# qiaobeibei/PPO-RL-Satellite

Hardware: NVIDIA B200
Metric: rk4_env_steps_per_sec (higher is better)
Workload: dtype f64

## Files before the change

### ppo-rl-satellite_b200/csrc/env_step.cu

```cuda
#include "sat_math.cuh"
#include "../../include/satb200.h"
#include <cmath>

namespace {

using namespace sat;

constexpr int kBlock = 128;
constexpr int kEnvsPerBlock = kBlock / 2;
constexpr int kFrontBlock = 64;
#ifndef SAT_FINISH_MINB
#define SAT_FINISH_MINB 7
#endif
constexpr int kFinishMinBlocks = SAT_FINISH_MINB;
constexpr int kObs = 18;
constexpr int kStatDims = 19;
constexpr int kWsHeader = 256;

SAT_DEV double shfl1(double v) { return __shfl_xor_sync(0xffffffffu, v, 1); }
SAT_DEV int shfl1(int v) { return __shfl_xor_sync(0xffffffffu, v, 1); }

SAT_DEV double clip16(double a) { return a < -1.6 ? -1.6 : (a > 1.6 ? 1.6 : a); }

__host__ __device__ inline int64_t ws_disprev_offset() { return kWsHeader; }
__host__ __device__ inline int64_t ws_partials_offset(int64_t n) { return kWsHeader + ((n * 8 + 255) / 256) * 256; }

struct Lane {
    double r[3], v[3];
    double a[3];
    double fuel_own;
    double dis_prev;
};

template <typename ActT>
SAT_DEV void load_and_gate(const SatEnvState& st, const SatEnvParams& p, const ActT* __restrict__ pa,
                           const ActT* __restrict__ ea, int64_t e, int craft, Lane& L, bool do_impulse,
                           const ActT* raw = nullptr ) {
// ... 40 lines not shown
#pragma unroll
    for (int k = 0; k < 3; ++k) { L.r[k] = y6[k]; L.v[k] = y6[3 + k]; }
}

SAT_DEV void propagate_rk4(const SatEnvParams& p, Lane& L) {
    double X[3], V[3];
#pragma unroll
    for (int k = 0; k < 3; ++k) { X[k] = p.r_cw[k] + L.r[k]; V[k] = p.v_cw[k] + L.v[k]; }
    const Rk4Consts c = make_rk4_consts(p.h, p.mu, p.re, p.j2);
    if (p.j2 != 0.0) {
#pragma unroll 1
        for (int s = 0; s < p.substeps; ++s) rk4_step<true>(X, V, c);
    } else {
#pragma unroll 1
        for (int s = 0; s < p.substeps; ++s) rk4_step<false>(X, V, c);
    }
#pragma unroll
    for (int k = 0; k < 3; ++k) { L.r[k] = X[k] - p.r_cw[k]; L.v[k] = V[k] - p.v_cw[k]; }
}

template <typename ActT, bool OBS>
__global__ void __launch_bounds__(kFrontBlock, 14)
env_front_rk4_kernel(const SatEnvState st, const ActT* __restrict__ pa, const ActT* __restrict__ ea,
                     double* __restrict__ dis_prev_out, float* __restrict__ obs_early,
                     float* __restrict__ pa_copy, float* __restrict__ ea_copy, const __grid_constant__ SatEnvParams p) {
    const int64_t tid = (int64_t)blockIdx.x * kFrontBlock + threadIdx.x;
    const int64_t env_raw = tid >> 1;
    const int craft = (int)(tid & 1);
    const bool valid = env_raw < st.n;
    const int64_t e = valid ? env_raw : st.n - 1;
    Lane L;
    if (OBS) {
        ActT raw[3];
        const ActT* act = craft ? ea : pa;
#pragma unroll
        for (int k = 0; k < 3; ++k) raw[k] = act[e * 3 + k];
        if (valid) {
            float* dc = craft ? ea_copy : pa_copy;
#pragma unroll
            for (int k = 0; k < 3; ++k) dc[e * 3 + k] = (float)raw[k];
        }
        load_and_gate(st, p, pa, ea, e, craft, L, true, raw);
    } else {
        load_and_gate(st, p, pa, ea, e, craft, L, true);
    }
    propagate_rk4(p, L);
    if (valid) {
        const int64_t ld = st.ld;
        const int base = craft * 6;
#pragma unroll
        for (int k = 0; k < 3; ++k) { st.state[(base + k) * ld + e] = L.r[k]; st.state[(base + 3 + k) * ld + e] = L.v[k]; }
        st.state[(SAT_COL_FUEL_C + craft) * ld + e] = L.fuel_own;
        if (craft == 0) dis_prev_out[e] = L.dis_prev;
    }
    if (OBS) {
        double P[3], Pv[3], E[3], Ev[3], d[3];
#pragma unroll
        for (int k = 0; k < 3; ++k) {
            const double o_r = shfl1(L.r[k]), o_v = shfl1(L.v[k]);
            P[k] = craft == 0 ? L.r[k] : o_r;  Pv[k] = craft == 0 ? L.v[k] : o_v;
            E[k] = craft == 0 ? o_r : L.r[k];  Ev[k] = craft == 0 ? o_v : L.v[k];
            d[k] = __dsub_rn(P[k], E[k]);
        }
        const double dis = norm3(d);
        const int count_new = st.istate[SAT_ICOL_COUNT * st.ld + e] + 1;
        const bool done = (dis <= p.d_capture) || (count_new >= p.max_episode_steps);
        if (done && p.auto_reset) {
#pragma unroll
            for (int k = 0; k < 3; ++k) { P[k] = p.reset_p[k]; E[k] = p.reset_e[k]; Pv[k] = 0.0; Ev[k] = 0.0; }
        }
        if (valid) {
            float* o = obs_early + e * kObs + craft * 9;
            if (craft == 0) {
#pragma unroll
                for (int k = 0; k < 3; ++k) { o[k] = (float)__dsub_rn(P[k], E[k]); o[3 + k] = (float)__dsub_rn(Pv[k], Ev[k]); o[6 + k] = (float)P[k]; }
            } else {
#pragma unroll
// ... 42 lines not shown
#endif
template <bool EXACT = true>
SAT_DEV void queue_run(SolveQueue& q) {
    const int total = q.count;
    int task = -1;
    Hybrd1<PFaiT<EXACT>> hs;
    if ((threadIdx.x >> 5) < SAT_SOLVE_WARPS)
    for (;;) {
        if (task < 0) {
            const int t = atomicAdd(&q.next, 1);
            if (t < total) {
                task = t;
                PFaiT<EXACT> f; f.A = q.A[t]; f.sth = q.sth[t]; f.dvm = q.dvm[t];
                hs.init_warm(f, dz_guess(q.guess[t]), q.trig[q.guess[t]]);
            } else task = total;
        }
        const bool active = task < total;
        if (!__any_sync(0xffffffffu, active)) break;
        if (active && hs.step()) { q.alpha[task] = hs.x; task = -1; }
    }
    __syncthreads();
}

template <bool FUSED, typename ActT, int MINB, bool EXACT>
__global__ void __launch_bounds__(kBlock, MINB)
env_step_kernel(const SatEnvState st, const ActT* __restrict__ pa, const ActT* __restrict__ ea,
                const int32_t* __restrict__ count_override, float* __restrict__ obs_f32,
                double* __restrict__ obs_f64, double* __restrict__ term_obs_f64,
                double* __restrict__ reward_out, uint8_t* __restrict__ done_out,
                const double* __restrict__ dis_prev_in, double* __restrict__ partials,
                unsigned int* __restrict__ ticket, const __grid_constant__ SatEnvParams p) {
    union SharedBlock { SolveQueue queue; double tile_term[kEnvsPerBlock][kObs]; __device__ SharedBlock() {} };
    __shared__ SharedBlock shm;
    __shared__ double tile[kEnvsPerBlock][kStatDims];
    SolveQueue& queue = shm.queue;
    double (&tile_term)[kEnvsPerBlock][kObs] = shm.tile_term;
    queue_init<EXACT>(queue);

    const int64_t tid = (int64_t)blockIdx.x * kBlock + threadIdx.x;
    const int64_t env_raw = tid >> 1;
    const int craft = (int)(tid & 1);
    const bool valid = env_raw < st.n;
    const int64_t e = valid ? env_raw : st.n - 1;
    const int64_t ld = st.ld;
    double* __restrict__ S = st.state;
    int32_t* __restrict__ I = st.istate;
    if (ticket && blockIdx.x == 0 && threadIdx.x == 0) *ticket = 0u;

    Lane L;
    load_and_gate(st, p, pa, ea, e, craft, L, FUSED);
    if (FUSED) propagate_cw(p, L);
    else L.dis_prev = dis_prev_in[e];
    const int dz_stale = I[SAT_ICOL_DZ * ld + e];
    const int count = I[SAT_ICOL_COUNT * ld + e];
    int err = I[SAT_ICOL_ERR * ld + e];
    const double ret = S[SAT_COL_RET * ld + e];

    double P[3], Pv[3], E[3], Ev[3], d[3];
#pragma unroll
    for (int k = 0; k < 3; ++k) {
        const double o_r = shfl1(L.r[k]), o_v = shfl1(L.v[k]);
        P[k] = craft == 0 ? L.r[k] : o_r;  Pv[k] = craft == 0 ? L.v[k] : o_v;
        E[k] = craft == 0 ? o_r : L.r[k];  Ev[k] = craft == 0 ? o_v : L.v[k];
        d[k] = __dsub_rn(P[k], E[k]);
    }
    const double dis = norm3(d);
    const int count_new = count_override ? count_override[e] : count + 1;
    const bool captured = dis <= p.d_capture;
    const bool timeout = count_new >= p.max_episode_steps;
    const bool done = captured || timeout;
    const double fuel_oth = shfl1(L.fuel_own);
    const double fuel_c = craft == 0 ? L.fuel_own : fuel_oth;
    double pa_gated[3];
#pragma unroll
    for (int k = 0; k < 3; ++k) { const double o = shfl1(L.a[k]); pa_gated[k] = craft == 0 ? L.a[k] : o; }

    const int le = threadIdx.x >> 1;
    const bool reset_now = done && p.auto_reset;
    const int64_t env0 = (int64_t)blockIdx.x * kEnvsPerBlock;
    const int64_t rem = st.n - env0;
    const int rows = (int)(rem < kEnvsPerBlock ? rem : kEnvsPerBlock);
    {
        double Po[3], Pvo[3], Eo[3], Evo[3];
#pragma unroll
        for (int k = 0; k < 3; ++k) {
            Po[k] = reset_now ? p.reset_p[k] : P[k];  Pvo[k] = reset_now ? 0.0 : Pv[k];
            Eo[k] = reset_now ? p.reset_e[k] : E[k];  Evo[k] = reset_now ? 0.0 : Ev[k];
        }
        if (craft == 0) {
#pragma unroll
            for (int k = 0; k < 3; ++k) { tile[le][k] = __dsub_rn(Po[k], Eo[k]); tile[le][3 + k] = __dsub_rn(Pvo[k], Evo[k]); tile[le][6 + k] = Po[k]; }
        } else {
#pragma unroll
            for (int k = 0; k < 3; ++k) { tile[le][9 + k] = Pvo[k]; tile[le][12 + k] = Eo[k]; tile[le][15 + k] = Evo[k]; }
        }
        __syncthreads();
        const int total = rows * kObs;
        for (int idx = threadIdx.x; idx < total; idx += kBlock) {
            const int row = idx / kObs, col = idx - row * kObs;
            const double val = tile[row][col];
            if (obs_f32) obs_f32[env0 * kObs + idx] = (float)val;
            if (obs_f64) obs_f64[env0 * kObs + idx] = val;
        }
    }

    const bool need_dz = !done && !p.skip_danger_zone && p.flag != 2;
    DzNode nd;
    {
        double Ri[3], Vi[3];
#pragma unroll
        for (int k = 0; k < 3; ++k) { Ri[k] = __dadd_rn(p.r_cw[k], L.r[k]); Vi[k] = __dadd_rn(p.v_cw[k], L.v[k]); }
        dz_prepare<EXACT>(craft, need_dz, Ri, Vi, fuel_c, p.u_grav, nd);
    }
    int slot0, slot1;
    double alpha0, alpha1;
    queue_push(queue, nd, slot0, slot1, alpha0, alpha1);
    queue_run<EXACT>(queue);
    if (slot0 >= 0) alpha0 = queue.alpha[slot0];
    if (slot1 >= 0) alpha1 = queue.alpha[slot1];
    __syncthreads();
    const int dz_eval = dz_finalize<EXACT>(need_dz, nd, alpha0, alpha1, nullptr);
    int dz_new = dz_stale;
    if (need_dz) {
        if (dz_eval >= 0) dz_new = dz_eval;
        else { dz_new = 0; err = 1; }
    }

    double reward = 0.0, cos_a = 0.0, cos_b = 0.0;
    if (p.flag == 2) reward = 0.0;
    else if (captured) reward = (p.flag == 0) ? 100.0 : -150.0;
    else if (timeout) reward = (p.flag == 0) ? 0.0 : 100.0;
    else {
        const bool pv4_on = pa_gated[0] != 0.0 && pa_gated[1] != 0.0 && pa_gated[2] != 0.0;
        double u1[3], w1[3], u2[3], w2[3];
#pragma unroll
        for (int k = 0; k < 3; ++k) {
            u1[k] = craft == 0 ? P[k] : d[k];   w1[k] = craft == 0 ? E[k] : Pv[k];
            u2[k] = craft == 0 ? Pv[k] : d[k];  w2[k] = craft == 0 ? Ev[k] : (pv4_on ? pa_gated[k] : Pv[k]);
        }
        const double ca = cosine3(u1, w1);
        double cb = cosine3(u2, w2);
        if (craft == 1) cb = pv4_on ? -cb : 0.0;
        cos_a = ca; cos_b = cb;
    }
    const double oth_a = shfl1(cos_a), oth_b = shfl1(cos_b);
    if (!captured && !timeout && p.flag != 2) {
        const double pv1 = craft == 0 ? cos_a : oth_a, pv2 = craft == 0 ? cos_b : oth_b;
        const double pv3 = craft == 0 ? oth_a : cos_a, pv4 = craft == 0 ? oth_b : cos_b;
        const double ra = (dis < L.dis_prev) ? 1.0 : -1.0;
        const double rb = (p.d_capture <= dis && dis <= 4.0 * p.d_capture) ? -1.0 : -2.0;
        const double rc = (dz_new == 0) ? -1.0 : dz_new * 0.5;
        double rr = __dadd_rn(__dadd_rn(ra, rb), rc);
        rr = __dadd_rn(rr, pv1);
        rr = __dadd_rn(rr, __dmul_rn(0.6, pv2));
        rr = __dadd_rn(rr, __dmul_rn(0.2, pv3));
        rr = __dadd_rn(rr, __dmul_rn(2.0, pv4));
        reward = (p.flag == 0) ? rr : -rr;
    }
    const double ret_new = __dadd_rn(__dmul_rn(p.gamma, ret), reward);

    if (term_obs_f64) {
        if (craft == 0) {
#pragma unroll
            for (int k = 0; k < 3; ++k) { tile_term[le][k] = d[k]; tile_term[le][3 + k] = __dsub_rn(Pv[k], Ev[k]); tile_term[le][6 + k] = P[k]; }
        } else {
#pragma unroll
            for (int k = 0; k < 3; ++k) { tile_term[le][9 + k] = Pv[k]; tile_term[le][12 + k] = E[k]; tile_term[le][15 + k] = Ev[k]; }
        }
    }

    int int_state_new = 0, count_store = count_new;
    if (reset_now) {
#pragma unroll
        for (int k = 0; k < 3; ++k) {
            P[k] = p.reset_p[k]; E[k] = p.reset_e[k]; Pv[k] = 0.0; Ev[k] = 0.0;
            L.r[k] = craft == 0 ? P[k] : E[k]; L.v[k] = 0.0;
        }
        int_state_new = 1; count_store = 0;
    }

    if (valid) {
        const int base = craft * 6;
        if (FUSED || reset_now) {
#pragma unroll
            for (int k = 0; k < 3; ++k) { S[(base + k) * ld + e] = L.r[k]; S[(base + 3 + k) * ld + e] = L.v[k]; }
        }
        if (FUSED) S[(SAT_COL_FUEL_C + craft) * ld + e] = L.fuel_own;
        if (craft == 0) {
            S[SAT_COL_DIS * ld + e] = dis;
            S[SAT_COL_RET * ld + e] = done ? 0.0 : ret_new;
            I[SAT_ICOL_DZ * ld + e] = dz_new;
            I[SAT_ICOL_COUNT * ld + e] = count_store;
            reward_out[e] = reward;
            done_out[e] = done ? 1 : 0;
        } else {
            I[SAT_ICOL_INTSTATE * ld + e] = int_state_new;
            I[SAT_ICOL_ERR * ld + e] = err;
        }
    }

    if (craft == 0) tile[le][18] = ret_new;
    __syncthreads();
    if (term_obs_f64) {
        const int total = rows * kObs;
        for (int idx = threadIdx.x; idx < total; idx += kBlock) {
            const int row = idx / kObs, col = idx - row * kObs;
            term_obs_f64[env0 * kObs + idx] = tile_term[row][col];
        }
    }
    if (partials && threadIdx.x < kStatDims) {
        const int dim = threadIdx.x;
        double sum = 0.0;
        for (int row = 0; row < rows; ++row) sum += tile[row][dim];
        const double mean = sum / rows;
        double m2 = 0.0;
        for (int row = 0; row < rows; ++row) { double t = tile[row][dim] - mean; m2 += t * t; }
        partials[((int64_t)blockIdx.x * kStatDims + dim) * 2 + 0] = mean;
        partials[((int64_t)blockIdx.x * kStatDims + dim) * 2 + 1] = m2;
    }
}

__global__ void __launch_bounds__(kBlock)
danger_zone_kernel(const double* __restrict__ rv, const double* __restrict__ dv, int64_t n, double u_grav,
                   int32_t* __restrict__ count_out, double* __restrict__ debug_out) {
    __shared__ SolveQueue queue;
    queue_init(queue);
    const int64_t tid = (int64_t)blockIdx.x * kBlock + threadIdx.x;
    const int64_t env_raw = tid >> 1;
    const int craft = (int)(tid & 1);
    const bool valid = env_raw < n;
    const int64_t e = valid ? env_raw : n - 1;
    double Ri[3], Vi[3];
#pragma unroll
    for (int k = 0; k < 3; ++k) { Ri[k] = rv[e * 12 + craft * 6 + k]; Vi[k] = rv[e * 12 + craft * 6 + 3 + k]; }
    DzNode nd;
    dz_prepare(craft, true, Ri, Vi, dv[e], u_grav, nd);
    int slot0, slot1;
    double alpha0, alpha1;
    queue_push(queue, nd, slot0, slot1, alpha0, alpha1);
    queue_run(queue);
    if (slot0 >= 0) alpha0 = queue.alpha[slot0];
    if (slot1 >= 0) alpha1 = queue.alpha[slot1];
    DzDebug dbg = {0, 0, 0, 0, 0, 0, 0, 0};
    const int dz = dz_finalize(true, nd, alpha0, alpha1, debug_out ? &dbg : nullptr);
// ... 181 lines not shown
        double P[3], Pv[3], E[3], Ev[3], o[kObs];
#pragma unroll
        for (int k = 0; k < 3; ++k) {
            P[k] = st.state[(SAT_COL_P + k) * ld + e]; Pv[k] = st.state[(SAT_COL_PV + k) * ld + e];
            E[k] = st.state[(SAT_COL_E + k) * ld + e]; Ev[k] = st.state[(SAT_COL_EV + k) * ld + e];
        }
#pragma unroll
        for (int k = 0; k < 3; ++k) {
            o[k] = __dsub_rn(P[k], E[k]); o[3 + k] = __dsub_rn(Pv[k], Ev[k]);
            o[6 + k] = P[k]; o[9 + k] = Pv[k]; o[12 + k] = E[k]; o[15 + k] = Ev[k];
        }
#pragma unroll
        for (int j = 0; j < kObs; ++j) {
            double v = o[j];
            if (obs_stats) v = (v - obs_stats[1 + j]) / (obs_stats[1 + 2 * kObs + j] + 1e-8);
            tile[threadIdx.x * kObs + j] = (float)v;
        }
    }
    __syncthreads();
    const int64_t rem = st.n - e0;
    const int total = (int)(rem < kObsNormEnvs ? rem : kObsNormEnvs) * kObs;
    for (int idx = threadIdx.x; idx < total; idx += kObsNormEnvs) obs_f32[e0 * kObs + idx] = tile[idx];
}

constexpr int kNormRows = 128;

__global__ void __launch_bounds__(kNormRows)
norm_partial_kernel(const double* __restrict__ x, int64_t n, int dim, double* __restrict__ partials,
                    unsigned int* __restrict__ ticket) {
    __shared__ double tile[kNormRows * 32];
    if (blockIdx.x == 0 && threadIdx.x == 0) *ticket = 0u;
    const int64_t row0 = (int64_t)blockIdx.x * kNormRows;
    const int64_t rem = n - row0;
    const int rows = (int)(rem < kNormRows ? rem : kNormRows);
    const int total = rows * dim;
    for (int idx = threadIdx.x; idx < total; idx += kNormRows) tile[idx] = x[row0 * dim + idx];
    __syncthreads();
    if (threadIdx.x < dim) {
        const int d = threadIdx.x;
        double sum = 0.0;
        for (int r = 0; r < rows; ++r) sum += tile[r * dim + d];
        const double mean = sum / rows;
        double m2 = 0.0;
        for (int r = 0; r < rows; ++r) { double t = tile[r * dim + d] - mean; m2 += t * t; }
        partials[((int64_t)blockIdx.x * dim + d) * 2 + 0] = mean;
        partials[((int64_t)blockIdx.x * dim + d) * 2 + 1] = m2;
    }
}
// ... 7 lines not shown
    const double y = (x[idx] - mean) / (sd + 1e-8);
    if (out64) out64[idx] = y;
    if (out32) out32[idx] = (float)y;
}

int check_state(const SatEnvState* st) {
    if (!st || !st->state || !st->istate) return SAT_ERR_NULL;
    if (st->n <= 0 || st->ld < st->n || (st->ld & 1)) return SAT_ERR_SIZE;
    if (((uintptr_t)st->state & 15) || ((uintptr_t)st->istate & 15)) return SAT_ERR_SIZE;
    return SAT_OK;
}

inline int launch_status() {
    cudaError_t e = cudaGetLastError();
    return e == cudaSuccess ? SAT_OK : (int)e;
}

}

extern "C" {

int64_t sat_workspace_bytes(int64_t n) {
    if (n <= 0) return kWsHeader;
    int64_t nb_env = (n + kEnvsPerBlock - 1) / kEnvsPerBlock;
    int64_t nb_norm = (n + kNormRows - 1) / kNormRows;
    int64_t a = nb_env * kStatDims * 2 * (int64_t)sizeof(double);
    int64_t b = nb_norm * 32 * 2 * (int64_t)sizeof(double);
    return ws_partials_offset(n) + (a > b ? a : b);
}

void sat_env_default_params(SatEnvParams* p) {
    if (!p) return;
    SatEnvParams q = {};
    q.mode = SAT_MODE_CW; q.flag = 0; q.max_episode_steps = 1000; q.auto_reset = 1;
    q.action_dtype = SAT_ACT_F32; q.substeps = 100; q.skip_danger_zone = 0;
    q.d_capture = 100000.0; q.d_range = 100000.0;
    q.gamma = 0.99;
    q.h = 1.0; q.mu = 3.986e14; q.re = 6378137.0; q.j2 = 0.00108263;
    q.r_cw[0] = 27098000.0; q.r_cw[1] = 32306000.0; q.r_cw[2] = 0.0;
    q.v_cw[0] = -2350.0; q.v_cw[1] = 1970.0; q.v_cw[2] = 0.0;
    q.u_grav = 3.986e14;
    q.reset_p[0] = 200000.0; q.reset_e[0] = 18000.0;
    *p = q;
}

int sat_env_init(const SatEnvState* st, double fuel_c, double fuel_t, const SatEnvParams* p, void* stream) {
    int rc = check_state(st);
    if (rc) return rc;
    if (!p) return SAT_ERR_NULL;
    const int threads = 256;
    const unsigned blocks = (unsigned)((st->n + threads - 1) / threads);
// ... 14 lines not shown
int sat_env_observe_norm(const SatEnvState* st, const double* obs_stats, float* obs_f32, void* stream) {
    int rc = check_state(st);
    if (rc) return rc;
    if (!obs_f32) return SAT_ERR_NULL;
    const unsigned blocks = (unsigned)((st->n + kObsNormEnvs - 1) / kObsNormEnvs);
    env_observe_norm_kernel<<<blocks, kObsNormEnvs, 0, (cudaStream_t)stream>>>(*st, obs_stats, obs_f32);
    return launch_status();
}

int sat_env_observe(const SatEnvState* st, float* obs_f32, double* obs_f64, void* stream) {
    int rc = check_state(st);
    if (rc) return rc;
    if (!obs_f32 && !obs_f64) return SAT_ERR_NULL;
    const int threads = 256;
    const int64_t total = st->n * kObs;
    const unsigned blocks = (unsigned)((total + threads - 1) / threads);
    env_observe_kernel<<<blocks, threads, 0, (cudaStream_t)stream>>>(*st, obs_f32, obs_f64);
    return launch_status();
}

}

namespace {
int env_step_impl(const SatEnvState* st, const void* pa, const void* ea, const int32_t* count_override,
                  float* obs_f32, double* obs_f64, double* term_obs_f64, double* reward, uint8_t* done,
                  double* obs_stats, double* ret_stats, double* ret_std_out, void* workspace,
                  const SatEnvParams* p, void* stream, cudaEvent_t* ev, float* obs_early = nullptr,
                  cudaEvent_t front_done = nullptr, float* pa_copy = nullptr, float* ea_copy = nullptr) {
    int rc = check_state(st);
    if (rc) return rc;
    if (!pa || !ea || !reward || !done || !p) return SAT_ERR_NULL;
    const bool want_stats = obs_stats || ret_stats;
    if ((want_stats || p->mode == SAT_MODE_RK4) && !workspace) return SAT_ERR_NULL;
    if (p->mode != SAT_MODE_CW && p->mode != SAT_MODE_RK4) return SAT_ERR_MODE;
    if (p->action_dtype != SAT_ACT_F32 && p->action_dtype != SAT_ACT_F64) return SAT_ERR_MODE;
    if (p->flag < 0 || p->flag > 2) return SAT_ERR_MODE;
    if (p->mode == SAT_MODE_RK4 && p->substeps < 1) return SAT_ERR_SIZE;
    if (workspace && ((uintptr_t)workspace & 15)) return SAT_ERR_SIZE;
    cudaStream_t s = (cudaStream_t)stream;
    const int64_t n = st->n;
    const int64_t nblocks = (n + kEnvsPerBlock - 1) / kEnvsPerBlock;
    char* ws = (char*)workspace;
    unsigned int* ticket = ws ? (unsigned int*)ws : nullptr;
    double* dis_prev = ws ? (double*)(ws + ws_disprev_offset()) : nullptr;
    double* partials = want_stats ? (double*)(ws + ws_partials_offset(n)) : nullptr;
    if (ev) cudaEventRecord(ev[0], s);
#define SAT_LAUNCH_FINISH(FUSED, T, ...)                                                                                   \
    do {                                                                                                                   \
        if (p->fast_libm) env_step_kernel<FUSED, T, kFinishMinBlocks, false><<<(unsigned)nblocks, kBlock, 0, s>>>(__VA_ARGS__); \
        else env_step_kernel<FUSED, T, kFinishMinBlocks, true><<<(unsigned)nblocks, kBlock, 0, s>>>(__VA_ARGS__);          \
    } while (0)
    if (p->mode == SAT_MODE_CW) {
        if (ev) cudaEventRecord(ev[1], s);
        if (p->action_dtype == SAT_ACT_F32)
            SAT_LAUNCH_FINISH(true, float, *st, (const float*)pa, (const float*)ea,
                count_override, obs_f32, obs_f64, term_obs_f64, reward, done, nullptr, partials, ticket, *p);
        else
            SAT_LAUNCH_FINISH(true, double, *st, (const double*)pa, (const double*)ea,
                count_override, obs_f32, obs_f64, term_obs_f64, reward, done, nullptr, partials, ticket, *p);
    } else {
        const int64_t fblocks = (2 * n + kFrontBlock - 1) / kFrontBlock;
        if (obs_early && (count_override || p->action_dtype != SAT_ACT_F32 || !pa_copy || !ea_copy)) return SAT_ERR_MODE;
        if (obs_early) {
            env_front_rk4_kernel<float, true><<<(unsigned)fblocks, kFrontBlock, 0, s>>>(*st, (const float*)pa, (const float*)ea,
                                                                                       dis_prev, obs_early, pa_copy, ea_copy, *p);
            if (front_done) cudaEventRecord(front_done, s);
            SAT_LAUNCH_FINISH(false, float, *st, pa_copy, ea_copy,
                count_override, obs_f32, obs_f64, term_obs_f64, reward, done, dis_prev, partials, ticket, *p);
        } else if (p->action_dtype == SAT_ACT_F32) {
            env_front_rk4_kernel<float, false><<<(unsigned)fblocks, kFrontBlock, 0, s>>>(*st, (const float*)pa, (const float*)ea, dis_prev, nullptr, nullptr, nullptr, *p);
            if (ev) cudaEventRecord(ev[1], s);
            SAT_LAUNCH_FINISH(false, float, *st, (const float*)pa, (const float*)ea,
                count_override, obs_f32, obs_f64, term_obs_f64, reward, done, dis_prev, partials, ticket, *p);
        } else {
            env_front_rk4_kernel<double, false><<<(unsigned)fblocks, kFrontBlock, 0, s>>>(*st, (const double*)pa, (const double*)ea, dis_prev, nullptr, nullptr, nullptr, *p);
            if (ev) cudaEventRecord(ev[1], s);
            SAT_LAUNCH_FINISH(false, double, *st, (const double*)pa, (const double*)ea,
                count_override, obs_f32, obs_f64, term_obs_f64, reward, done, dis_prev, partials, ticket, *p);
        }
    }
#undef SAT_LAUNCH_FINISH
    rc = launch_status();
    if (rc) return rc;
    if (ev) cudaEventRecord(ev[2], s);
    if (partials) {
        stats_merge_kernel<<<kStatDims, kMergeThreads, 0, s>>>(partials, nblocks, n, kEnvsPerBlock, kStatDims,
                                                               obs_stats, kObs, ret_stats, ret_std_out, ticket);
        rc = launch_status();
    }
    if (ev) cudaEventRecord(ev[3], s);
    return rc;
}
}

extern "C" {

int sat_env_step(const SatEnvState* st, const void* pa, const void* ea, const int32_t* count_override,
                 float* obs_f32, double* obs_f64, double* term_obs_f64, double* reward, uint8_t* done,
                 double* obs_stats, double* ret_stats, double* ret_std_out, void* workspace,
                 const SatEnvParams* p, void* stream) {
    return env_step_impl(st, pa, ea, count_override, obs_f32, obs_f64, term_obs_f64, reward, done, obs_stats, ret_stats,
                         ret_std_out, workspace, p, stream, nullptr);
}

int sat_env_step_timed(const SatEnvState* st, const void* pa, const void* ea, const int32_t* count_override,
// ... 188 lines not shown
```

Baseline: 332.1 million.

## Split env step into setup, grid-wide danger-zone solve, and finish kernels with PDL

Replaces the single per-block finish kernel, which solved danger-zone root-finding in a block-local queue, with three kernels. A setup kernel writes observations and stats and pushes solve tasks into a global queue. A grid-wide solve kernel claims tasks in chunks across all blocks, and a finish kernel computes rewards and terminal outputs. Programmatic dependent launch lets kernel prologues overlap with their predecessors. The intent is to balance the irregular Newton-solve work across the whole GPU instead of per block, at the cost of extra global workspace traffic, kernel launches and a mandatory workspace.

```diff
diff --git a/ppo-rl-satellite_b200/csrc/env_step.cu b/ppo-rl-satellite_b200/csrc/env_step.cu
--- a/ppo-rl-satellite_b200/csrc/env_step.cu
+++ b/ppo-rl-satellite_b200/csrc/env_step.cu
@@ -1,6 +1,7 @@
 #include "sat_math.cuh"
 #include "../../include/satb200.h"
 #include <cmath>
+#include <type_traits>
 
 namespace {
 
@@ -9,10 +10,24 @@
 constexpr int kBlock = 128;
 constexpr int kEnvsPerBlock = kBlock / 2;
 constexpr int kFrontBlock = 64;
+#ifndef SAT_SETUP_MINB
+#define SAT_SETUP_MINB 7
+#endif
+#ifndef SAT_SOLVE_MINB
+#define SAT_SOLVE_MINB 3
+#endif
+#ifndef SAT_SOLVE_CLAIM
+#define SAT_SOLVE_CLAIM 16
+#endif
 #ifndef SAT_FINISH_MINB
-#define SAT_FINISH_MINB 7
+#define SAT_FINISH_MINB 8
 #endif
+constexpr int kSetupMinBlocks = SAT_SETUP_MINB;
+constexpr int kSolveBlock = 256;
+constexpr int kSolveMinBlocks = SAT_SOLVE_MINB;
+constexpr int kSolveClaim = SAT_SOLVE_CLAIM;
 constexpr int kFinishMinBlocks = SAT_FINISH_MINB;
+constexpr int kNormRows = 128;
 constexpr int kObs = 18;
 constexpr int kStatDims = 19;
 constexpr int kWsHeader = 256;
@@ -99,7 +114,7 @@
 template <typename ActT, bool OBS>
 __global__ void __launch_bounds__(kFrontBlock, 14)
 env_front_rk4_kernel(const SatEnvState st, const ActT* __restrict__ pa, const ActT* __restrict__ ea,
-                     double* __restrict__ dis_prev_out, float* __restrict__ obs_early,
+                     double* __restrict__ dis_prev_out, unsigned int* __restrict__ dz_counters, float* __restrict__ obs_early,
                      float* __restrict__ pa_copy, float* __restrict__ ea_copy, const __grid_constant__ SatEnvParams p) {
     const int64_t tid = (int64_t)blockIdx.x * kFrontBlock + threadIdx.x;
     const int64_t env_raw = tid >> 1;
@@ -130,6 +145,7 @@
         st.state[(SAT_COL_FUEL_C + craft) * ld + e] = L.fuel_own;
         if (craft == 0) dis_prev_out[e] = L.dis_prev;
     }
+    if (tid == 0) { dz_counters[0] = 0u; dz_counters[1] = 0u; }
     if (OBS) {
         double P[3], Pv[3], E[3], Ev[3], d[3];
 #pragma unroll
@@ -218,21 +234,219 @@
     __syncthreads();
 }
 
-template <bool FUSED, typename ActT, int MINB, bool EXACT>
-__global__ void __launch_bounds__(kBlock, MINB)
-env_step_kernel(const SatEnvState st, const ActT* __restrict__ pa, const ActT* __restrict__ ea,
-                const int32_t* __restrict__ count_override, float* __restrict__ obs_f32,
-                double* __restrict__ obs_f64, double* __restrict__ term_obs_f64,
-                double* __restrict__ reward_out, uint8_t* __restrict__ done_out,
-                const double* __restrict__ dis_prev_in, double* __restrict__ partials,
-                unsigned int* __restrict__ ticket, const __grid_constant__ SatEnvParams p) {
-    union SharedBlock { SolveQueue queue; double tile_term[kEnvsPerBlock][kObs]; __device__ SharedBlock() {} };
-    __shared__ SharedBlock shm;
-    __shared__ double tile[kEnvsPerBlock][kStatDims];
-    SolveQueue& queue = shm.queue;
-    double (&tile_term)[kEnvsPerBlock][kObs] = shm.tile_term;
-    queue_init<EXACT>(queue);
-
+struct __align__(16) DzTask { double A, sth, dvm; int guess, pad; };
+
+struct DzWork {
+    unsigned int* count;
+    unsigned int* next;
+    DzTask* task;
+    double* alpha;
+    double *r_c, *sq_e_sin, *sq_k, *dvm, *sth, *cth, *r_ft;
+    int *status, *slot0, *slot1;
+};
+
+inline int64_t al256(int64_t b) { return (b + 255) / 256 * 256; }
+inline int64_t ws_partials_bytes(int64_t n) {
+    const int64_t nb_env = (n + kEnvsPerBlock - 1) / kEnvsPerBlock, nb_norm = (n + kNormRows - 1) / kNormRows;
+    const int64_t a = nb_env * kStatDims * 2 * (int64_t)sizeof(double), b = nb_norm * 32 * 2 * (int64_t)sizeof(double);
+    return a > b ? a : b;
+}
+inline int64_t ws_dz(int64_t n, char* ws, DzWork* w) {
+    const int64_t q = 4 * n, lanes = 2 * n;
+    const int64_t bytes[12] = {q * (int64_t)sizeof(DzTask), q * 8, lanes * 8, lanes * 8, lanes * 8, lanes * 8, lanes * 8,
+                               lanes * 8, lanes * 8, lanes * 4, lanes * 4, lanes * 4};
+    char* at[12];
+    int64_t off = ws_partials_offset(n) + al256(ws_partials_bytes(n));
+    for (int i = 0; i < 12; ++i) { at[i] = ws ? ws + off : nullptr; off += al256(bytes[i]); }
+    if (w) {
+        w->count = (unsigned int*)(ws + 4); w->next = (unsigned int*)(ws + 8);
+        w->task = (DzTask*)at[0]; w->alpha = (double*)at[1];
+        w->r_c = (double*)at[2]; w->sq_e_sin = (double*)at[3]; w->sq_k = (double*)at[4]; w->dvm = (double*)at[5];
+        w->sth = (double*)at[6]; w->cth = (double*)at[7]; w->r_ft = (double*)at[8];
+        w->status = (int*)at[9]; w->slot0 = (int*)at[10]; w->slot1 = (int*)at[11];
+    }
+    return off;
+}
+
+SAT_DEV void griddep_wait() { asm volatile("griddepcontrol.wait;" ::: "memory"); }
+SAT_DEV void griddep_launch_dependents() { asm volatile("griddepcontrol.launch_dependents;" ::: "memory"); }
+
+template <bool FUSED, typename ActT, bool EXACT>
+__global__ void __launch_bounds__(kBlock, kSetupMinBlocks)
+env_dz_setup_kernel(const SatEnvState st, const ActT* __restrict__ pa, const ActT* __restrict__ ea,
+                    const int32_t* __restrict__ count_override, float* __restrict__ obs_f32, double* __restrict__ obs_f64,
+                    double* __restrict__ dis_prev, double* __restrict__ partials, const DzWork w,
+                    const __grid_constant__ SatEnvParams p) {
+    griddep_launch_dependents();
+    __shared__ double tile[kEnvsPerBlock][kObs];
+    const int64_t tid = (int64_t)blockIdx.x * kBlock + threadIdx.x;
+    const int64_t env_raw = tid >> 1;
+    const int craft = (int)(tid & 1);
+    const bool valid = env_raw < st.n;
+    const int64_t e = valid ? env_raw : st.n - 1;
+    const int64_t ld = st.ld;
+    double* __restrict__ S = st.state;
+    const int32_t* __restrict__ I = st.istate;
+
+    Lane L;
+    const int base = craft * 6;
+    if (FUSED) {
+        load_and_gate(st, p, pa, ea, e, craft, L, true);
+        propagate_cw(p, L);
+        if (valid) {
+#pragma unroll
+            for (int k = 0; k < 3; ++k) { S[(base + k) * ld + e] = L.r[k]; S[(base + 3 + k) * ld + e] = L.v[k]; }
+            S[(SAT_COL_FUEL_C + craft) * ld + e] = L.fuel_own;
+            if (craft == 0) dis_prev[e] = L.dis_prev;
+        }
+    } else {
+#pragma unroll
+        for (int k = 0; k < 3; ++k) { L.r[k] = S[(base + k) * ld + e]; L.v[k] = S[(base + 3 + k) * ld + e]; }
+        L.fuel_own = S[(SAT_COL_FUEL_C + craft) * ld + e];
+    }
+    const int count = I[SAT_ICOL_COUNT * ld + e];
+
+    double P[3], Pv[3], E[3], Ev[3], d[3];
+#pragma unroll
+    for (int k = 0; k < 3; ++k) {
+        const double o_r = shfl1(L.r[k]), o_v = shfl1(L.v[k]);
+        P[k] = craft == 0 ? L.r[k] : o_r;  Pv[k] = craft == 0 ? L.v[k] : o_v;
+        E[k] = craft == 0 ? o_r : L.r[k];  Ev[k] = craft == 0 ? o_v : L.v[k];
+        d[k] = __dsub_rn(P[k], E[k]);
+    }
+    const double dis = norm3(d);
+    const int count_new = count_override ? count_override[e] : count + 1;
+    const bool done = (dis <= p.d_capture) || (count_new >= p.max_episode_steps);
+    const double fuel_oth = shfl1(L.fuel_own);
+    const double fuel_c = craft == 0 ? L.fuel_own : fuel_oth;
+
+    const int le = threadIdx.x >> 1;
+    const bool reset_now = done && p.auto_reset;
+    const int64_t env0 = (int64_t)blockIdx.x * kEnvsPerBlock;
+    const int64_t rem = st.n - env0;
+    const int rows = (int)(rem < kEnvsPerBlock ? rem : kEnvsPerBlock);
+    {
+        double Po[3], Pvo[3], Eo[3], Evo[3];
+#pragma unroll
+        for (int k = 0; k < 3; ++k) {
+            Po[k] = reset_now ? p.reset_p[k] : P[k];  Pvo[k] = reset_now ? 0.0 : Pv[k];
+            Eo[k] = reset_now ? p.reset_e[k] : E[k];  Evo[k] = reset_now ? 0.0 : Ev[k];
+        }
+        if (craft == 0) {
+#pragma unroll
+            for (int k = 0; k < 3; ++k) { tile[le][k] = __dsub_rn(Po[k], Eo[k]); tile[le][3 + k] = __dsub_rn(Pvo[k], Evo[k]); tile[le][6 + k] = Po[k]; }
+        } else {
+#pragma unroll
+            for (int k = 0; k < 3; ++k) { tile[le][9 + k] = Pvo[k]; tile[le][12 + k] = Eo[k]; tile[le][15 + k] = Evo[k]; }
+        }
+        __syncthreads();
+        const int total = rows * kObs;
+        for (int idx = threadIdx.x; idx < total; idx += kBlock) {
+            const int row = idx / kObs, col = idx - row * kObs;
+            const double val = tile[row][col];
+            if (obs_f32) obs_f32[env0 * kObs + idx] = (float)val;
+            if (obs_f64) obs_f64[env0 * kObs + idx] = val;
+        }
+        if (partials && threadIdx.x < kObs) {
+            const int dim = threadIdx.x;
+            double sum = 0.0;
+            for (int row = 0; row < rows; ++row) sum += tile[row][dim];
+            const double mean = sum / rows;
+            double m2 = 0.0;
+            for (int row = 0; row < rows; ++row) { double t = tile[row][dim] - mean; m2 += t * t; }
+            partials[((int64_t)blockIdx.x * kStatDims + dim) * 2 + 0] = mean;
+            partials[((int64_t)blockIdx.x * kStatDims + dim) * 2 + 1] = m2;
+        }
+    }
+
+    const bool need_dz = !done && !p.skip_danger_zone && p.flag != 2;
+    DzNode nd;
+    {
+        double Ri[3], Vi[3];
+#pragma unroll
+        for (int k = 0; k < 3; ++k) { Ri[k] = __dadd_rn(p.r_cw[k], L.r[k]); Vi[k] = __dadd_rn(p.v_cw[k], L.v[k]); }
+        dz_prepare<EXACT>(craft, need_dz, Ri, Vi, fuel_c, p.u_grav, nd);
+    }
+    const bool q0 = valid && nd.status == 2 && !dz_degenerate(nd.A0, nd.sth, nd.dvm);
+    const bool q1 = valid && nd.status == 2 && !dz_degenerate(nd.A1, nd.sth, nd.dvm);
+    const unsigned b0 = __ballot_sync(0xffffffffu, q0), b1 = __ballot_sync(0xffffffffu, q1);
+    const unsigned lt = (1u << (threadIdx.x & 31)) - 1u;
+    const int in_warp = __popc(b0) + __popc(b1);
+    unsigned int first = 0;
+    if (in_warp && (threadIdx.x & 31) == 0) first = atomicAdd(w.count, (unsigned int)in_warp);
+    int slot = (int)__shfl_sync(0xffffffffu, first, 0) + __popc(b0 & lt) + __popc(b1 & lt);
+    int slot0 = -1, slot1 = -1;
+    if (q0) { slot0 = slot++; w.task[slot0] = DzTask{nd.A0, nd.sth, nd.dvm, 0, 0}; }
+    if (q1) { slot1 = slot; w.task[slot1] = DzTask{nd.A1, nd.sth, nd.dvm, 1, 0}; }
+    if (valid) {
+        const int64_t li = 2 * e + craft;
+        w.status[li] = nd.status;
+        if (nd.status >= 1) w.r_ft[li] = nd.r_ft;
+        if (nd.status == 2) {
+            w.r_c[li] = nd.r_c; w.sq_e_sin[li] = nd.sq_e_sin; w.sq_k[li] = nd.sq_k;
+            w.dvm[li] = nd.dvm; w.sth[li] = nd.sth; w.cth[li] = nd.cth;
+            w.slot0[li] = slot0; w.slot1[li] = slot1;
+        }
+    }
+}
+
+template <bool EXACT>
+__global__ void __launch_bounds__(kSolveBlock, kSolveMinBlocks)
+env_dz_solve_kernel(const DzWork w) {
+    __shared__ double trig[2][4];
+    if (threadIdx.x < 4) {
+        const int j = threadIdx.x >> 1, k = threadIdx.x & 1;
+        const double x0 = dz_guess(j);
+        const double h = 1.4901161193847656e-08 * fabs(x0);
+        const double2 sc = Lm<EXACT>::sincos(k ? x0 + h : x0);
+        trig[j][2 * k] = sc.x; trig[j][2 * k + 1] = sc.y;
+    }
+    __syncthreads();
+    griddep_wait();
+    griddep_launch_dependents();
+    const int total = (int)*w.count;
+    const int lane = threadIdx.x & 31;
+    const unsigned lt = (1u << lane) - 1u;
+    int task = -1;
+    int cur = 0, end = 0;
+    bool drained = false;
+    Hybrd1<PFaiT<EXACT>> hs;
+    for (;;) {
+        unsigned need = __ballot_sync(0xffffffffu, task < 0);
+        while (need) {
+            if (cur >= end) {
+                unsigned int c = (unsigned int)total;
+                if (!drained && lane == 0) c = atomicAdd(w.next, (unsigned int)kSolveClaim);
+                cur = (int)min(__shfl_sync(0xffffffffu, c, 0), (unsigned int)total);
+                end = min(cur + kSolveClaim, total);
+                if (cur == total) { drained = true; if (task < 0) task = total; break; }
+            }
+            const int t = cur + __popc(need & lt);
+            if (task < 0 && t < end) {
+                task = t;
+                const DzTask q = w.task[t];
+                PFaiT<EXACT> f; f.A = q.A; f.sth = q.sth; f.dvm = q.dvm;
+                hs.init_warm(f, dz_guess(q.guess), trig[q.guess]);
+            }
+            cur = min(cur + __popc(need), end);
+            need = __ballot_sync(0xffffffffu, task < 0);
+        }
+        const bool active = task < total;
+        if (!__any_sync(0xffffffffu, active)) break;
+        if (active && hs.step()) { w.alpha[task] = hs.x; task = -1; }
+    }
+}
+
+template <bool FUSED, typename ActT, bool EXACT>
+__global__ void __launch_bounds__(kBlock, kFinishMinBlocks)
+env_finish_kernel(const SatEnvState st, const ActT* __restrict__ pa, const ActT* __restrict__ ea,
+                  const int32_t* __restrict__ count_override, double* __restrict__ term_obs_f64,
+                  double* __restrict__ reward_out, uint8_t* __restrict__ done_out, const double* __restrict__ dis_prev_in,
+                  double* __restrict__ partials, unsigned int* __restrict__ ticket, const DzWork w,
+                  const __grid_constant__ SatEnvParams p) {
+    __shared__ double tile_term[kEnvsPerBlock][kObs];
+    __shared__ double ret_col[kEnvsPerBlock];
+    if (FUSED) griddep_wait();
     const int64_t tid = (int64_t)blockIdx.x * kBlock + threadIdx.x;
     const int64_t env_raw = tid >> 1;
     const int craft = (int)(tid & 1);
@@ -241,12 +455,10 @@
     const int64_t ld = st.ld;
     double* __restrict__ S = st.state;
     int32_t* __restrict__ I = st.istate;
-    if (ticket && blockIdx.x == 0 && threadIdx.x == 0) *ticket = 0u;
 
     Lane L;
-    load_and_gate(st, p, pa, ea, e, craft, L, FUSED);
-    if (FUSED) propagate_cw(p, L);
-    else L.dis_prev = dis_prev_in[e];
+    load_and_gate(st, p, pa, ea, e, craft, L, false);
+    L.dis_prev = dis_prev_in[e];
     const int dz_stale = I[SAT_ICOL_DZ * ld + e];
     const int count = I[SAT_ICOL_COUNT * ld + e];
     int err = I[SAT_ICOL_ERR * ld + e];
@@ -265,56 +477,64 @@
     const bool captured = dis <= p.d_capture;
     const bool timeout = count_new >= p.max_episode_steps;
     const bool done = captured || timeout;
-    const double fuel_oth = shfl1(L.fuel_own);
-    const double fuel_c = craft == 0 ? L.fuel_own : fuel_oth;
     double pa_gated[3];
 #pragma unroll
     for (int k = 0; k < 3; ++k) { const double o = shfl1(L.a[k]); pa_gated[k] = craft == 0 ? L.a[k] : o; }
-
     const int le = threadIdx.x >> 1;
     const bool reset_now = done && p.auto_reset;
     const int64_t env0 = (int64_t)blockIdx.x * kEnvsPerBlock;
     const int64_t rem = st.n - env0;
     const int rows = (int)(rem < kEnvsPerBlock ? rem : kEnvsPerBlock);
-    {
-        double Po[3], Pvo[3], Eo[3], Evo[3];
+
+    double cos_a = 0.0, cos_b = 0.0;
+    if (p.flag != 2 && !captured && !timeout) {
+        const bool pv4_on = pa_gated[0] != 0.0 && pa_gated[1] != 0.0 && pa_gated[2] != 0.0;
+        double u1[3], w1[3], u2[3], w2[3];
 #pragma unroll
         for (int k = 0; k < 3; ++k) {
-            Po[k] = reset_now ? p.reset_p[k] : P[k];  Pvo[k] = reset_now ? 0.0 : Pv[k];
-            Eo[k] = reset_now ? p.reset_e[k] : E[k];  Evo[k] = reset_now ? 0.0 : Ev[k];
-        }
+            u1[k] = craft == 0 ? P[k] : d[k];   w1[k] = craft == 0 ? E[k] : Pv[k];
+            u2[k] = craft == 0 ? Pv[k] : d[k];  w2[k] = craft == 0 ? Ev[k] : (pv4_on ? pa_gated[k] : Pv[k]);
+        }
+        const double ca = cosine3(u1, w1);
+        double cb = cosine3(u2, w2);
+        if (craft == 1) cb = pv4_on ? -cb : 0.0;
+        cos_a = ca; cos_b = cb;
+    }
+    const double oth_a = shfl1(cos_a), oth_b = shfl1(cos_b);
+
+    if (term_obs_f64) {
         if (craft == 0) {
 #pragma unroll
-            for (int k = 0; k < 3; ++k) { tile[le][k] = __dsub_rn(Po[k], Eo[k]); tile[le][3 + k] = __dsub_rn(Pvo[k], Evo[k]); tile[le][6 + k] = Po[k]; }
+            for (int k = 0; k < 3; ++k) { tile_term[le][k] = d[k]; tile_term[le][3 + k] = __dsub_rn(Pv[k], Ev[k]); tile_term[le][6 + k] = P[k]; }
         } else {
 #pragma unroll
-            for (int k = 0; k < 3; ++k) { tile[le][9 + k] = Pvo[k]; tile[le][12 + k] = Eo[k]; tile[le][15 + k] = Evo[k]; }
+            for (int k = 0; k < 3; ++k) { tile_term[le][9 + k] = Pv[k]; tile_term[le][12 + k] = E[k]; tile_term[le][15 + k] = Ev[k]; }
         }
         __syncthreads();
         const int total = rows * kObs;
         for (int idx = threadIdx.x; idx < total; idx += kBlock) {
             const int row = idx / kObs, col = idx - row * kObs;
-            const double val = tile[row][col];
-            if (obs_f32) obs_f32[env0 * kObs + idx] = (float)val;
-            if (obs_f64) obs_f64[env0 * kObs + idx] = val;
-        }
-    }
-
+            term_obs_f64[env0 * kObs + idx] = tile_term[row][col];
+        }
+    }
+
+    if (!FUSED) griddep_wait();
+    if (ticket && blockIdx.x == 0 && threadIdx.x == 0) *ticket = 0u;
     const bool need_dz = !done && !p.skip_danger_zone && p.flag != 2;
+    const int64_t li = 2 * e + craft;
     DzNode nd;
-    {
-        double Ri[3], Vi[3];
-#pragma unroll
-        for (int k = 0; k < 3; ++k) { Ri[k] = __dadd_rn(p.r_cw[k], L.r[k]); Vi[k] = __dadd_rn(p.v_cw[k], L.v[k]); }
-        dz_prepare<EXACT>(craft, need_dz, Ri, Vi, fuel_c, p.u_grav, nd);
-    }
-    int slot0, slot1;
-    double alpha0, alpha1;
-    queue_push(queue, nd, slot0, slot1, alpha0, alpha1);
-    queue_run<EXACT>(queue);
-    if (slot0 >= 0) alpha0 = queue.alpha[slot0];
-    if (slot1 >= 0) alpha1 = queue.alpha[slot1];
-    __syncthreads();
+    nd.u = p.u_grav; nd.status = w.status[li];
+    nd.r_c = 0.0; nd.sq_e_sin = 0.0; nd.sq_k = 0.0; nd.dvm = 0.0; nd.sth = 0.0; nd.cth = 1.0; nd.r_ft = 0.0;
+    nd.A0 = 0.0; nd.A1 = 0.0; nd.theta = 0.0; nd.f_cx = 0.0;
+    double alpha0 = dz_guess(0), alpha1 = dz_guess(1);
+    if (nd.status >= 1) nd.r_ft = w.r_ft[li];
+    if (nd.status == 2) {
+        nd.r_c = w.r_c[li]; nd.sq_e_sin = w.sq_e_sin[li]; nd.sq_k = w.sq_k[li];
+        nd.dvm = w.dvm[li]; nd.sth = w.sth[li]; nd.cth = w.cth[li];
+        const int slot0 = w.slot0[li], slot1 = w.slot1[li];
+        if (slot0 >= 0) alpha0 = w.alpha[slot0];
+        if (slot1 >= 0) alpha1 = w.alpha[slot1];
+    }
     const int dz_eval = dz_finalize<EXACT>(need_dz, nd, alpha0, alpha1, nullptr);
     int dz_new = dz_stale;
     if (need_dz) {
@@ -322,25 +542,11 @@
         else { dz_new = 0; err = 1; }
     }
 
-    double reward = 0.0, cos_a = 0.0, cos_b = 0.0;
+    double reward = 0.0;
     if (p.flag == 2) reward = 0.0;
     else if (captured) reward = (p.flag == 0) ? 100.0 : -150.0;
     else if (timeout) reward = (p.flag == 0) ? 0.0 : 100.0;
     else {
-        const bool pv4_on = pa_gated[0] != 0.0 && pa_gated[1] != 0.0 && pa_gated[2] != 0.0;
-        double u1[3], w1[3], u2[3], w2[3];
-#pragma unroll
-        for (int k = 0; k < 3; ++k) {
-            u1[k] = craft == 0 ? P[k] : d[k];   w1[k] = craft == 0 ? E[k] : Pv[k];
-            u2[k] = craft == 0 ? Pv[k] : d[k];  w2[k] = craft == 0 ? Ev[k] : (pv4_on ? pa_gated[k] : Pv[k]);
-        }
-        const double ca = cosine3(u1, w1);
-        double cb = cosine3(u2, w2);
-        if (craft == 1) cb = pv4_on ? -cb : 0.0;
-        cos_a = ca; cos_b = cb;
-    }
-    const double oth_a = shfl1(cos_a), oth_b = shfl1(cos_b);
-    if (!captured && !timeout && p.flag != 2) {
         const double pv1 = craft == 0 ? cos_a : oth_a, pv2 = craft == 0 ? cos_b : oth_b;
         const double pv3 = craft == 0 ? oth_a : cos_a, pv4 = craft == 0 ? oth_b : cos_b;
         const double ra = (dis < L.dis_prev) ? 1.0 : -1.0;
@@ -355,67 +561,39 @@
     }
     const double ret_new = __dadd_rn(__dmul_rn(p.gamma, ret), reward);
 
-    if (term_obs_f64) {
-        if (craft == 0) {
-#pragma unroll
-            for (int k = 0; k < 3; ++k) { tile_term[le][k] = d[k]; tile_term[le][3 + k] = __dsub_rn(Pv[k], Ev[k]); tile_term[le][6 + k] = P[k]; }
-        } else {
-#pragma unroll
-            for (int k = 0; k < 3; ++k) { tile_term[le][9 + k] = Pv[k]; tile_term[le][12 + k] = E[k]; tile_term[le][15 + k] = Ev[k]; }
-        }
-    }
-
-    int int_state_new = 0, count_store = count_new;
-    if (reset_now) {
-#pragma unroll
-        for (int k = 0; k < 3; ++k) {
-            P[k] = p.reset_p[k]; E[k] = p.reset_e[k]; Pv[k] = 0.0; Ev[k] = 0.0;
-            L.r[k] = craft == 0 ? P[k] : E[k]; L.v[k] = 0.0;
-        }
-        int_state_new = 1; count_store = 0;
-    }
-
     if (valid) {
         const int base = craft * 6;
-        if (FUSED || reset_now) {
-#pragma unroll
-            for (int k = 0; k < 3; ++k) { S[(base + k) * ld + e] = L.r[k]; S[(base + 3 + k) * ld + e] = L.v[k]; }
-        }
-        if (FUSED) S[(SAT_COL_FUEL_C + craft) * ld + e] = L.fuel_own;
+        if (reset_now) {
+#pragma unroll
+            for (int k = 0; k < 3; ++k) { S[(base + k) * ld + e] = craft == 0 ? p.reset_p[k] : p.reset_e[k]; S[(base + 3 + k) * ld + e] = 0.0; }
+        }
         if (craft == 0) {
             S[SAT_COL_DIS * ld + e] = dis;
             S[SAT_COL_RET * ld + e] = done ? 0.0 : ret_new;
             I[SAT_ICOL_DZ * ld + e] = dz_new;
-            I[SAT_ICOL_COUNT * ld + e] = count_store;
+            I[SAT_ICOL_COUNT * ld + e] = reset_now ? 0 : count_new;
             reward_out[e] = reward;
             done_out[e] = done ? 1 : 0;
         } else {
-            I[SAT_ICOL_INTSTATE * ld + e] = int_state_new;
+            I[SAT_ICOL_INTSTATE * ld + e] = reset_now ? 1 : 0;
             I[SAT_ICOL_ERR * ld + e] = err;
         }
     }
 
-    if (craft == 0) tile[le][18] = ret_new;
-    __syncthreads();
-    if (term_obs_f64) {
-        const int total = rows * kObs;
-        for (int idx = threadIdx.x; idx < total; idx += kBlock) {
-            const int row = idx / kObs, col = idx - row * kObs;
-            term_obs_f64[env0 * kObs + idx] = tile_term[row][col];
-        }
-    }
-    if (partials && threadIdx.x < kStatDims) {
-        const int dim = threadIdx.x;
-        double sum = 0.0;
-        for (int row = 0; row < rows; ++row) sum += tile[row][dim];
-        const double mean = sum / rows;
-        double m2 = 0.0;
-        for (int row = 0; row < rows; ++row) { double t = tile[row][dim] - mean; m2 += t * t; }
-        partials[((int64_t)blockIdx.x * kStatDims + dim) * 2 + 0] = mean;
-        partials[((int64_t)blockIdx.x * kStatDims + dim) * 2 + 1] = m2;
-    }
-}
-
+    if (partials) {
+        if (craft == 0) ret_col[le] = ret_new;
+        __syncthreads();
+        if (threadIdx.x == 0) {
+            double sum = 0.0;
+            for (int row = 0; row < rows; ++row) sum += ret_col[row];
+            const double mean = sum / rows;
+            double m2 = 0.0;
+            for (int row = 0; row < rows; ++row) { double t = ret_col[row] - mean; m2 += t * t; }
+            partials[((int64_t)blockIdx.x * kStatDims + kObs) * 2 + 0] = mean;
+            partials[((int64_t)blockIdx.x * kStatDims + kObs) * 2 + 1] = m2;
+        }
+    }
+}
 __global__ void __launch_bounds__(kBlock)
 danger_zone_kernel(const double* __restrict__ rv, const double* __restrict__ dv, int64_t n, double u_grav,
                    int32_t* __restrict__ count_out, double* __restrict__ debug_out) {
@@ -643,8 +821,6 @@
     const int total = (int)(rem < kObsNormEnvs ? rem : kObsNormEnvs) * kObs;
     for (int idx = threadIdx.x; idx < total; idx += kObsNormEnvs) obs_f32[e0 * kObs + idx] = tile[idx];
 }
-
-constexpr int kNormRows = 128;
 
 __global__ void __launch_bounds__(kNormRows)
 norm_partial_kernel(const double* __restrict__ x, int64_t n, int dim, double* __restrict__ partials,
@@ -698,11 +874,7 @@
 
 int64_t sat_workspace_bytes(int64_t n) {
     if (n <= 0) return kWsHeader;
-    int64_t nb_env = (n + kEnvsPerBlock - 1) / kEnvsPerBlock;
-    int64_t nb_norm = (n + kNormRows - 1) / kNormRows;
-    int64_t a = nb_env * kStatDims * 2 * (int64_t)sizeof(double);
-    int64_t b = nb_norm * 32 * 2 * (int64_t)sizeof(double);
-    return ws_partials_offset(n) + (a > b ? a : b);
+    return ws_dz(n, nullptr, nullptr);
 }
 
 void sat_env_default_params(SatEnvParams* p) {
@@ -763,6 +935,66 @@
 }
 
 namespace {
+template <typename... KArgs, typename... Args>
+int launch_pdl(void (*kernel)(KArgs...), unsigned blocks, int threads, cudaStream_t s, Args... args) {
+    cudaLaunchConfig_t cfg = {};
+    cfg.gridDim = dim3(blocks); cfg.blockDim = dim3(threads); cfg.stream = s;
+    cudaLaunchAttribute attr[1];
+    attr[0].id = cudaLaunchAttributeProgrammaticStreamSerialization;
+    attr[0].val.programmaticStreamSerializationAllowed = 1;
+    cfg.attrs = attr; cfg.numAttrs = 1;
+    const cudaError_t e = cudaLaunchKernelEx(&cfg, kernel, args...);
+    return e == cudaSuccess ? launch_status() : (int)e;
+}
+
+template <bool EXACT>
+int solve_blocks(int64_t n, unsigned* blocks) {
+    static int resident[64] = {0};
+    int dev = 0;
+    cudaError_t e = cudaGetDevice(&dev);
+    if (e != cudaSuccess) return (int)e;
+    int r = (dev >= 0 && dev < 64) ? resident[dev] : 0;
+    if (r <= 0) {
+        int sms = 0, per_sm = 0;
+        if ((e = cudaDeviceGetAttribute(&sms, cudaDevAttrMultiProcessorCount, dev)) != cudaSuccess) return (int)e;
+        if ((e = cudaOccupancyMaxActiveBlocksPerMultiprocessor(&per_sm, env_dz_solve_kernel<EXACT>, kSolveBlock, 0)) != cudaSuccess)
+            return (int)e;
+        r = sms * (per_sm > 0 ? per_sm : 1);
+        if (dev >= 0 && dev < 64) resident[dev] = r;
+    }
+    const int64_t need = (4 * n + kSolveBlock - 1) / kSolveBlock;
+    *blocks = (unsigned)(need < r ? need : r);
+    return SAT_OK;
+}
+
+template <bool FUSED, typename ActT, bool EXACT>
+int launch_back_half(const SatEnvState& st, const ActT* pa, const ActT* ea, const int32_t* count_override, float* obs_f32,
+                     double* obs_f64, double* term_obs_f64, double* reward, uint8_t* done, double* dis_prev,
+                     double* partials, unsigned int* ticket, const DzWork& w, const SatEnvParams& p, cudaStream_t s) {
+    const unsigned nblocks = (unsigned)((st.n + kEnvsPerBlock - 1) / kEnvsPerBlock);
+    using SetupT = std::conditional_t<FUSED, ActT, float>;
+    env_dz_setup_kernel<FUSED, SetupT, EXACT><<<nblocks, kBlock, 0, s>>>(st, (const SetupT*)pa, (const SetupT*)ea, count_override,
+                                                                           obs_f32, obs_f64, dis_prev, partials, w, p);
+    int rc = launch_status();
+    if (rc) return rc;
+    unsigned sblocks = 0;
+    if ((rc = solve_blocks<EXACT>(st.n, &sblocks))) return rc;
+    if ((rc = launch_pdl(env_dz_solve_kernel<EXACT>, sblocks, kSolveBlock, s, w))) return rc;
+    return launch_pdl(env_finish_kernel<FUSED, ActT, EXACT>, nblocks, kBlock, s, st, pa, ea, count_override, term_obs_f64,
+                      reward, done, (const double*)dis_prev, partials, ticket, w, p);
+}
+
+template <bool FUSED, typename ActT>
+int launch_back_half(bool exact, const SatEnvState& st, const void* pa, const void* ea, const int32_t* count_override,
+                     float* obs_f32, double* obs_f64, double* term_obs_f64, double* reward, uint8_t* done, double* dis_prev,
+                     double* partials, unsigned int* ticket, const DzWork& w, const SatEnvParams& p, cudaStream_t s) {
+    if (exact)
+        return launch_back_half<FUSED, ActT, true>(st, (const ActT*)pa, (const ActT*)ea, count_override, obs_f32, obs_f64,
+                                                   term_obs_f64, reward, done, dis_prev, partials, ticket, w, p, s);
+    return launch_back_half<FUSED, ActT, false>(st, (const ActT*)pa, (const ActT*)ea, count_override, obs_f32, obs_f64,
+                                                term_obs_f64, reward, done, dis_prev, partials, ticket, w, p, s);
+}
+
 int env_step_impl(const SatEnvState* st, const void* pa, const void* ea, const int32_t* count_override,
                   float* obs_f32, double* obs_f64, double* term_obs_f64, double* reward, uint8_t* done,
                   double* obs_stats, double* ret_stats, double* ret_std_out, void* workspace,
@@ -771,57 +1003,57 @@
     int rc = check_state(st);
     if (rc) return rc;
     if (!pa || !ea || !reward || !done || !p) return SAT_ERR_NULL;
-    const bool want_stats = obs_stats || ret_stats;
-    if ((want_stats || p->mode == SAT_MODE_RK4) && !workspace) return SAT_ERR_NULL;
     if (p->mode != SAT_MODE_CW && p->mode != SAT_MODE_RK4) return SAT_ERR_MODE;
     if (p->action_dtype != SAT_ACT_F32 && p->action_dtype != SAT_ACT_F64) return SAT_ERR_MODE;
     if (p->flag < 0 || p->flag > 2) return SAT_ERR_MODE;
     if (p->mode == SAT_MODE_RK4 && p->substeps < 1) return SAT_ERR_SIZE;
-    if (workspace && ((uintptr_t)workspace & 15)) return SAT_ERR_SIZE;
+    if (!workspace) return SAT_ERR_NULL;
+    if ((uintptr_t)workspace & 15) return SAT_ERR_SIZE;
     cudaStream_t s = (cudaStream_t)stream;
     const int64_t n = st->n;
     const int64_t nblocks = (n + kEnvsPerBlock - 1) / kEnvsPerBlock;
     char* ws = (char*)workspace;
-    unsigned int* ticket = ws ? (unsigned int*)ws : nullptr;
-    double* dis_prev = ws ? (double*)(ws + ws_disprev_offset()) : nullptr;
-    double* partials = want_stats ? (double*)(ws + ws_partials_offset(n)) : nullptr;
+    unsigned int* ticket = (unsigned int*)ws;
+    double* dis_prev = (double*)(ws + ws_disprev_offset());
+    double* partials = (obs_stats || ret_stats) ? (double*)(ws + ws_partials_offset(n)) : nullptr;
+    DzWork w;
+    ws_dz(n, ws, &w);
+    const bool exact = !p->fast_libm;
     if (ev) cudaEventRecord(ev[0], s);
-#define SAT_LAUNCH_FINISH(FUSED, T, ...)                                                                                   \
-    do {                                                                                                                   \
-        if (p->fast_libm) env_step_kernel<FUSED, T, kFinishMinBlocks, false><<<(unsigned)nblocks, kBlock, 0, s>>>(__VA_ARGS__); \
-        else env_step_kernel<FUSED, T, kFinishMinBlocks, true><<<(unsigned)nblocks, kBlock, 0, s>>>(__VA_ARGS__);          \
-    } while (0)
     if (p->mode == SAT_MODE_CW) {
+        cudaError_t ce = cudaMemsetAsync(w.count, 0, 2 * sizeof(unsigned int), s);
+        if (ce != cudaSuccess) return (int)ce;
         if (ev) cudaEventRecord(ev[1], s);
         if (p->action_dtype == SAT_ACT_F32)
-            SAT_LAUNCH_FINISH(true, float, *st, (const float*)pa, (const float*)ea,
-                count_override, obs_f32, obs_f64, term_obs_f64, reward, done, nullptr, partials, ticket, *p);
+            rc = launch_back_half<true, float>(exact, *st, pa, ea, count_override, obs_f32, obs_f64, term_obs_f64, reward,
+                                               done, dis_prev, partials, ticket, w, *p, s);
         else
-            SAT_LAUNCH_FINISH(true, double, *st, (const double*)pa, (const double*)ea,
-                count_override, obs_f32, obs_f64, term_obs_f64, reward, done, nullptr, partials, ticket, *p);
+            rc = launch_back_half<true, double>(exact, *st, pa, ea, count_override, obs_f32, obs_f64, term_obs_f64, reward,
+                                                done, dis_prev, partials, ticket, w, *p, s);
     } else {
         const int64_t fblocks = (2 * n + kFrontBlock - 1) / kFrontBlock;
         if (obs_early && (count_override || p->action_dtype != SAT_ACT_F32 || !pa_copy || !ea_copy)) return SAT_ERR_MODE;
         if (obs_early) {
             env_front_rk4_kernel<float, true><<<(unsigned)fblocks, kFrontBlock, 0, s>>>(*st, (const float*)pa, (const float*)ea,
-                                                                                       dis_prev, obs_early, pa_copy, ea_copy, *p);
+                                                                                       dis_prev, w.count, obs_early, pa_copy, ea_copy, *p);
             if (front_done) cudaEventRecord(front_done, s);
-            SAT_LAUNCH_FINISH(false, float, *st, pa_copy, ea_copy,
-                count_override, obs_f32, obs_f64, term_obs_f64, reward, done, dis_prev, partials, ticket, *p);
+            if ((rc = launch_status())) return rc;
+            rc = launch_back_half<false, float>(exact, *st, pa_copy, ea_copy, count_override, obs_f32, obs_f64, term_obs_f64,
+                                                reward, done, dis_prev, partials, ticket, w, *p, s);
         } else if (p->action_dtype == SAT_ACT_F32) {
-            env_front_rk4_kernel<float, false><<<(unsigned)fblocks, kFrontBlock, 0, s>>>(*st, (const float*)pa, (const float*)ea, dis_prev, nullptr, nullptr, nullptr, *p);
+            env_front_rk4_kernel<float, false><<<(unsigned)fblocks, kFrontBlock, 0, s>>>(*st, (const float*)pa, (const float*)ea, dis_prev, w.count, nullptr, nullptr, nullptr, *p);
             if (ev) cudaEventRecord(ev[1], s);
-            SAT_LAUNCH_FINISH(false, float, *st, (const float*)pa, (const float*)ea,
-                count_override, obs_f32, obs_f64, term_obs_f64, reward, done, dis_prev, partials, ticket, *p);
+            if ((rc = launch_status())) return rc;
+            rc = launch_back_half<false, float>(exact, *st, pa, ea, count_override, obs_f32, obs_f64, term_obs_f64, reward,
+                                                done, dis_prev, partials, ticket, w, *p, s);
         } else {
-            env_front_rk4_kernel<double, false><<<(unsigned)fblocks, kFrontBlock, 0, s>>>(*st, (const double*)pa, (const double*)ea, dis_prev, nullptr, nullptr, nullptr, *p);
+            env_front_rk4_kernel<double, false><<<(unsigned)fblocks, kFrontBlock, 0, s>>>(*st, (const double*)pa, (const double*)ea, dis_prev, w.count, nullptr, nullptr, nullptr, *p);
             if (ev) cudaEventRecord(ev[1], s);
-            SAT_LAUNCH_FINISH(false, double, *st, (const double*)pa, (const double*)ea,
-                count_override, obs_f32, obs_f64, term_obs_f64, reward, done, dis_prev, partials, ticket, *p);
-        }
-    }
-#undef SAT_LAUNCH_FINISH
-    rc = launch_status();
+            if ((rc = launch_status())) return rc;
+            rc = launch_back_half<false, double>(exact, *st, pa, ea, count_override, obs_f32, obs_f64, term_obs_f64, reward,
+                                                 done, dis_prev, partials, ticket, w, *p, s);
+        }
+    }
     if (rc) return rc;
     if (ev) cudaEventRecord(ev[2], s);
     if (partials) {
```

Measured after the change: 338.0 million (median of 6 runs). 1.8% higher.
